# saidwivedi/TokenHMR

Measured on NVIDIA H100. Metric: images/sec (256x192) at bs=64 per GPU, full TokenHMR forward, higher is better.
Workload: dtype f16 operands / f32 accumulate

## Files before the change

tokenhmr_b200/_build.py:

```python
from __future__ import annotations

import hashlib
import os
import subprocess
import sys
from pathlib import Path

PKG_DIR = Path(__file__).resolve().parent
CSRC = PKG_DIR / "csrc"
LIB_PATH = PKG_DIR / "libtokenhmr_b200.so"
STAMP = PKG_DIR / ".libtokenhmr_b200.stamp"
PROBE_SRC = PKG_DIR.parent / "tests" / "csrc" / "kernel_probe.cu"
PROBE_PATH = PKG_DIR.parent / "tests" / "libthmr_probe.so"
PROBE_STAMP = PKG_DIR.parent / "tests" / ".libthmr_probe.stamp"
GEMM_PROBE_SRC = PKG_DIR.parent / "tests" / "csrc" / "gemm_probe.cu"
GEMM_PROBE_PATH = PKG_DIR.parent / "tests" / "libthmr_gemm_probe.so"
GEMM_PROBE_STAMP = PKG_DIR.parent / "tests" / ".libthmr_gemm_probe.stamp"

NVCC_FLAGS = [
    "-gencode", "arch=compute_90a,code=sm_90a",
    "-lineinfo", "-O3", "-std=c++17",
    "--expt-relaxed-constexpr",
    "-Xcompiler", "-fPIC", "-shared",
]
PROBE_FLAGS = ["-Xcompiler", "-fvisibility=hidden"]


def _nvcc() -> str:
    for cand in (os.environ.get("NVCC"), "/usr/local/cuda/bin/nvcc", "nvcc"):
        if cand and (os.path.isabs(cand) and os.path.exists(cand) or not os.path.isabs(cand)):
            return cand
    return "nvcc"


def source_hash(probe: bool = False) -> str:
    h = hashlib.sha256()
    files = sorted(CSRC.glob("*.cu")) + sorted(CSRC.glob("*.cuh")) + sorted((PKG_DIR.parent / "include").glob("*.h"))
    if probe:
        files += sorted(PROBE_SRC.parent.glob("*.cu"))
    for f in files:
# ... 3 lines not shown
    return h.hexdigest()


def _compile(src: Path, out: Path, stamp: Path, flags: list, want: str, force: bool, verbose: bool) -> Path:
    if not force and out.exists() and stamp.exists() and stamp.read_text().strip() == want:
        return out
    cmd = [_nvcc(), *flags, "-o", str(out), str(src)]
    if verbose:
        cmd.insert(1, "-Xptxas=-v")
        print(" ".join(cmd), file=sys.stderr)
    res = subprocess.run(cmd, capture_output=True, text=True)
    if res.returncode != 0:
        raise RuntimeError(f"nvcc failed ({res.returncode}):\n{res.stdout}\n{res.stderr}")
    if verbose:
        print(res.stderr, file=sys.stderr)
    stamp.write_text(want)
    return out


def build_probe(force: bool = False, verbose: bool = False) -> Path:
    if GEMM_PROBE_SRC.exists():
        _compile(GEMM_PROBE_SRC, GEMM_PROBE_PATH, GEMM_PROBE_STAMP, NVCC_FLAGS + PROBE_FLAGS, source_hash(probe=True),
                 force, verbose)
    return _compile(PROBE_SRC, PROBE_PATH, PROBE_STAMP, NVCC_FLAGS + PROBE_FLAGS, source_hash(probe=True), force,
                    verbose)


def build(force: bool = False, verbose: bool = False) -> Path:
    path = _compile(CSRC / "tokenhmr_b200.cu", LIB_PATH, STAMP, NVCC_FLAGS, source_hash(), force, verbose)
    if PROBE_SRC.exists():
        build_probe(force, verbose)
    return path


if __name__ == "__main__":
    print(build(force="--force" in sys.argv, verbose="-v" in sys.argv))
```

tokenhmr_b200/csrc/gemm_host.cuh:

```cuda
#pragma once
#include "common.cuh"

#include "gemm_wgmma.cuh"

namespace thmr {

struct GemmPlan {
  CUtensorMap tmA, tmB;
  CUtensorMap tmC;
  GemmParams p;
  int bn;
  int grid;
  int cluster;
  int fp8;
  int epi;
};

struct GemmDesc {
  const __half* A; int lda; long long a_rows;
  const __half* B; int ldb;
  int M, N, K;
  const float* bias = nullptr;
  const float* resid = nullptr; int ldr = 0; int resid_mod = 0;
  int act = kActNone; int act32 = 0;
  float* out32 = nullptr; int ld32 = 0;
  __half* out16 = nullptr; int ld16 = 0;
  int taps = 1; int cin = 0; int tap_row0 = 0; int tap_stride = 0;
  int seq_pitch = 0, seq_lo = 0, seq_hi = 0;
  float alpha = 1.0f;
  long long* argmin_out = nullptr; const float* row_sq = nullptr; const float* col_sq = nullptr;
  int* screen_rows = nullptr; int* screen_count = nullptr; const float* screen_cmax2 = nullptr;
  float screen_rel = 0.f, screen_abs = 0.f; int screen_row0 = 0;
  const int* row_map = nullptr; const int* m_dev = nullptr; int m_dev_off = 0;
  int force_bn = 0;
  int force_epi = 0;
  unsigned long long* stamp = nullptr;
  int fp8 = 0;
  const float* a_scale = nullptr; int ld_as = 0;
  const float* w_scale = nullptr;
  uint8_t* out8 = nullptr; int ld8 = 0; float* out8_scale = nullptr; int ld8s = 0;
};

inline int pick_bn(int M, int N, int K, bool staged_epilogue, int epi_kind, int force) {
  if (force) return force;
  const int sms = num_sms();
  const int tm = (M + kGemmBM - 1) / kGemmBM;
  const int num_kb = (K + kGemmBK - 1) / kGemmBK;
  int best = 256;
  double best_cost = -1;
  const int cands[4] = {256, 128, 64, 32};
  for (int i = 0; i < 4; ++i) {
    const int bn = cands[i];
    const long tiles = static_cast<long>(tm) * ((N + bn - 1) / bn);
    const long waves = (tiles + sms - 1) / sms;
    const double mma = 4.0 * bn;
    const double feed = (128.0 + bn) * 128.0 / 32.0;
    const double epilogue = !staged_epilogue                                 ? 0.0
                            : bn >= 128 && gemm_epi_tma_store(epi_kind)       ? 2500.0 * bn / 128
                            : bn >= 128 && epi_kind == kEpiBiasResidF32       ? 9000.0 * bn / 128
                            : bn == 256                                       ? 55000.0
                                                                              : 7000.0 * bn / 128;
    const double cost = waves * (num_kb * ((mma > feed ? mma : feed) + 40.0) + epilogue);
    if (best_cost < 0 || cost < best_cost) { best_cost = cost; best = bn; }
  }
  return best;
}

inline int pick_bn_fp8(int M, int N, int K) {
  const int sms = num_sms();
  const int tm = (M + kGemmBM - 1) / kGemmBM;
  const int num_kb = (K + 127) / 128;
  int best = 128;
  double best_cost = -1;
  const int cands[2] = {128, 64};
  for (int i = 0; i < 2; ++i) {
    const int bn = cands[i];
    const long tiles = static_cast<long>(tm) * ((N + bn - 1) / bn);
    const long waves = (tiles + sms - 1) / sms;
    const double mma = 4.0 * bn;
    const double feed = (128.0 + bn) * 128.0 / 32.0;
    const double cost = waves * (num_kb * ((mma > feed ? mma : feed) + bn + 40.0) + 7000.0 * bn / 128);
    if (best_cost < 0 || cost < best_cost) { best_cost = cost; best = bn; }
  }
  return best;
}

inline int gemm_pick_epi(const GemmDesc& d, int bn, int cluster) {
  auto al16 = [](const void* q) { return (reinterpret_cast<uintptr_t>(q) & 15) == 0; };
// ... 25 lines not shown
  THMR_CHECK(d.ld_as >= m_pad && d.ld_as % 4 == 0 && (reinterpret_cast<uintptr_t>(d.a_scale) & 15) == 0,
             "gemm fp8: activation scales need a 16-byte aligned [K/128][>= %ld] layout (ld_as %d)", m_pad, d.ld_as);
  int bn = d.force_bn ? d.force_bn : d.out8 ? 128 : pick_bn_fp8(d.M, d.N, d.K);
  THMR_CHECK(bn == 64 || bn == 128, "gemm fp8: block_n %d (64 or 128)", bn);
  THMR_CHECK(!d.out8 || (bn == 128 && d.out8_scale && d.ld8s >= d.M && !d.resid && !d.act32 && !d.seq_pitch),
             "gemm fp8: e4m3 output needs block_n 128, its scale array and no residual / mask / act32");
  GemmParams& p = plan->p;
  memset(&p, 0, sizeof(p));
  p.M = d.M; p.N = d.N; p.K = d.K;
  p.out32 = d.out32; p.ld32 = d.ld32; p.out16 = d.out16; p.ld16 = d.ld16;
  p.bias = d.bias; p.resid = d.resid; p.ldr = d.ldr; p.resid_mod = d.resid_mod; p.act = d.act; p.act32 = d.act32;
  p.seq_pitch = d.seq_pitch; p.seq_lo = d.seq_lo; p.seq_hi = d.seq_hi;
  p.alpha = d.alpha;
  p.stamp = d.stamp;
  p.kblocks_per_tap = d.K / 128;
  p.a_scale = d.a_scale; p.ld_as = d.ld_as; p.w_scale = d.w_scale;
  p.out8 = d.out8; p.ld8 = d.ld8; p.out8_scale = d.out8_scale; p.ld8s = d.ld8s;
  THMR_TRY(make_tmap_2d_e4m3(&plan->tmA, d.A, d.a_rows, d.K, d.lda, kGemmBM, 128));
  THMR_TRY(make_tmap_2d_e4m3(&plan->tmB, d.B, d.N, d.K, d.ldb, bn, 128));
  memset(&plan->tmC, 0, sizeof(plan->tmC));
  THMR_CHECK(d.force_epi == 0 || d.force_epi == 1 + kEpiGeneral, "gemm fp8: general epilogue only");
  plan->bn = bn;
  plan->cluster = 1;
  plan->fp8 = 1;
  plan->epi = kEpiGeneral;
  const long tiles_m = (d.M + kGemmBM - 1) / kGemmBM;
  const long tiles = tiles_m * ((d.N + bn - 1) / bn);
  p.m_fast = (tiles_m > 1 && d.M < d.N) ? 1 : 0;
  const long slots = num_sms();
  plan->grid = static_cast<int>(tiles < slots ? tiles : slots);
  return THMR_OK;
}

inline int gemm_make_plan(const GemmDesc& d, GemmPlan* plan) {
  if (d.fp8) return gemm_make_plan_fp8(d, plan);
  THMR_CHECK(d.M > 0 && d.N > 0 && d.K > 0, "gemm: bad shape %dx%dx%d", d.M, d.N, d.K);
  THMR_CHECK(d.out32 || d.out16 || d.argmin_out, "gemm: no output");
  const int cluster = d.force_bn == 512 ? 2 : 1;
  THMR_CHECK(cluster == 1 || !d.argmin_out, "gemm: block_n 512 (CTA pair) does not support the arg-min modes");
  const int kind = gemm_pick_epi(d, 256, cluster);
  const int bn = cluster == 2 ? 256 : pick_bn(d.M, d.N, d.K, d.argmin_out == nullptr, kind, d.force_bn);
  THMR_CHECK(bn == 32 || bn == 64 || bn == 128 || bn == 256, "gemm: bad block_n %d", bn);
  GemmParams& p = plan->p;
  memset(&p, 0, sizeof(p));
  p.M = d.M; p.N = d.N; p.K = d.K;
  p.out32 = d.out32; p.ld32 = d.ld32; p.out16 = d.out16; p.ld16 = d.ld16;
  p.bias = d.bias; p.resid = d.resid; p.ldr = d.ldr; p.resid_mod = d.resid_mod; p.act = d.act; p.act32 = d.act32;
  p.seq_pitch = d.seq_pitch; p.seq_lo = d.seq_lo; p.seq_hi = d.seq_hi;
  p.alpha = d.alpha; p.argmin_out = d.argmin_out; p.row_sq = d.row_sq; p.col_sq = d.col_sq;
  THMR_CHECK(!d.screen_rows || (d.argmin_out && d.screen_count && d.screen_cmax2),
             "gemm: screened arg-min needs its queue");
  THMR_CHECK((!d.m_dev && !d.row_map) || d.argmin_out, "gemm: device row count / row map are arg-min options");
  p.screen_rows = d.screen_rows; p.screen_count = d.screen_count; p.screen_cmax2 = d.screen_cmax2;
  p.screen_rel = d.screen_rel; p.screen_abs = d.screen_abs; p.screen_row0 = d.screen_row0;
  p.row_map = d.row_map; p.m_dev = d.m_dev; p.m_dev_off = d.m_dev_off;
  p.stamp = d.stamp;
  const int num_kb = (d.K + kGemmBK - 1) / kGemmBK;
  uint64_t a_cols = d.K;
  if (d.taps > 1) {
    THMR_CHECK(d.cin % kGemmBK == 0 && d.K == d.taps * d.cin, "gemm conv: cin %d taps %d K %d", d.cin, d.taps, d.K);
    p.kblocks_per_tap = d.cin / kGemmBK;
    p.tap_row0 = d.tap_row0; p.tap_stride = d.tap_stride;
    a_cols = d.cin;
  } else {
    p.kblocks_per_tap = num_kb;
  }
  THMR_TRY(make_tmap_2d_f16(&plan->tmA, d.A, d.a_rows, a_cols, d.lda, kGemmBM, kGemmBK, CU_TENSOR_MAP_SWIZZLE_128B));
  THMR_TRY(make_tmap_2d_f16(&plan->tmB, d.B, d.N, d.K, d.ldb, bn / cluster, kGemmBK, CU_TENSOR_MAP_SWIZZLE_128B));
  plan->bn = bn;
  plan->cluster = cluster;
  plan->fp8 = 0;
  plan->epi = gemm_pick_epi(d, bn, cluster);
  THMR_CHECK(d.force_epi == 0 || d.force_epi - 1 == kEpiGeneral || d.force_epi - 1 == plan->epi,
             "gemm: epilogue kind %d does not fit this GEMM (its kind is %d)", d.force_epi - 1, plan->epi);
  if (d.force_epi) plan->epi = d.force_epi - 1;
  memset(&plan->tmC, 0, sizeof(plan->tmC));
  if (gemm_epi_tma_store(plan->epi))
    THMR_TRY(make_tmap_2d_f16(&plan->tmC, d.out16, d.M, d.N, d.ld16, 64, 64, CU_TENSOR_MAP_SWIZZLE_128B));
  if (plan->epi == kEpiBiasResidF32)
    THMR_TRY(make_tmap_2d(&plan->tmC, CU_TENSOR_MAP_DATA_TYPE_FLOAT32, 4, d.out32, d.M, d.N, d.ld32, 64, 32,
                          CU_TENSOR_MAP_SWIZZLE_128B));
  const long tiles_m = (d.M + kGemmBM * cluster - 1) / (kGemmBM * cluster);
  const long tiles = d.argmin_out ? tiles_m : tiles_m * ((d.N + bn - 1) / bn);
  p.m_fast = (!d.argmin_out && tiles_m > 1 && d.M < d.N) ? 1 : 0;
  const long slots = num_sms() / cluster;
  plan->grid = cluster * static_cast<int>(tiles < slots ? tiles : slots);
  return THMR_OK;
}

template <int BN, int STAGES, int CLUSTER = 1, bool FP8 = false, int EPI = kEpiGeneral, bool TIMELINE = false>
inline int gemm_launch_t(const GemmPlan& plan, cudaStream_t stream) {
  using S = GemmSmem<BN, STAGES, FP8, EPI>;
  static_assert(S::kTotal <= kGemmSmemLimit, "GEMM shared memory exceeds 227 KB");
  static bool configured = false;
  if (!configured) {
    THMR_CUDA(cudaFuncSetAttribute(gemm_f16_tn_kernel<BN, STAGES, CLUSTER, FP8, EPI, TIMELINE>, cudaFuncAttributeMaxDynamicSharedMemorySize,
                                   S::kTotal));
    configured = true;
  }
  cudaLaunchConfig_t cfg = {};
  cfg.gridDim = dim3(plan.grid);
  cfg.blockDim = dim3(kGemmThreads);
  cfg.dynamicSmemBytes = S::kTotal;
  cfg.stream = stream;
  cudaLaunchAttribute attr[1];
  attr[0].id = cudaLaunchAttributeClusterDimension;
  attr[0].val.clusterDim.x = CLUSTER;
  attr[0].val.clusterDim.y = 1;
  attr[0].val.clusterDim.z = 1;
  cfg.attrs = attr;
  cfg.numAttrs = 1;
  THMR_CUDA(cudaLaunchKernelEx(&cfg, gemm_f16_tn_kernel<BN, STAGES, CLUSTER, FP8, EPI, TIMELINE>, plan.tmA, plan.tmB,
                               plan.tmC, plan.p));
  return THMR_OK;
}

template <int BN, int EPI>
constexpr int gemm_stages() {
  return BN == 256 ? 4 : EPI == kEpiBiasResidF32 ? 5 : 6;
}

template <int BN, bool TIMELINE>
inline int gemm_launch_epi(const GemmPlan& plan, cudaStream_t stream) {
  switch (plan.epi) {
    case kEpiGeneral: return gemm_launch_t<BN, gemm_stages<BN, kEpiGeneral>(), 1, false, kEpiGeneral, TIMELINE>(plan, stream);
    case kEpiF16: return gemm_launch_t<BN, gemm_stages<BN, kEpiF16>(), 1, false, kEpiF16, TIMELINE>(plan, stream);
    case kEpiBiasF16: return gemm_launch_t<BN, gemm_stages<BN, kEpiBiasF16>(), 1, false, kEpiBiasF16, TIMELINE>(plan, stream);
    case kEpiBiasGeluF16:
      return gemm_launch_t<BN, gemm_stages<BN, kEpiBiasGeluF16>(), 1, false, kEpiBiasGeluF16, TIMELINE>(plan, stream);
    case kEpiBiasResidF32:
      return gemm_launch_t<BN, gemm_stages<BN, kEpiBiasResidF32>(), 1, false, kEpiBiasResidF32, TIMELINE>(plan, stream);
  }
  return fail(THMR_ERR_INVALID, "gemm: unsupported epilogue kind %d", plan.epi);
}

inline int gemm_launch_plain(const GemmPlan& plan, cudaStream_t stream) {
  if (plan.fp8) {
    if (plan.bn == 128) return gemm_launch_t<128, 5, 1, true>(plan, stream);
    if (plan.bn == 64) return gemm_launch_t<64, 7, 1, true>(plan, stream);
    return fail(THMR_ERR_INVALID, "gemm fp8: unsupported block_n %d", plan.bn);
  }
  if (plan.cluster == 2) return gemm_launch_t<256, 4, 2>(plan, stream);
  switch (plan.bn) {
    case 256: return gemm_launch_epi<256, false>(plan, stream);
    case 128: return gemm_launch_epi<128, false>(plan, stream);
    case 64: return gemm_launch_t<64, 8>(plan, stream);
    case 32: return gemm_launch_t<32, 8>(plan, stream);
  }
  return fail(THMR_ERR_INVALID, "gemm: unsupported block_n %d", plan.bn);
}

template <bool TIMELINE = false>
inline int gemm_launch(const GemmPlan& plan, cudaStream_t stream) {
  if constexpr (TIMELINE) {
    THMR_CHECK(!plan.fp8 && plan.cluster == 1 && (plan.bn == 128 || plan.bn == 256),
               "gemm timeline: fp16 block_n 128 / 256 only (block_n %d)", plan.bn);
    return plan.bn == 256 ? gemm_launch_epi<256, true>(plan, stream) : gemm_launch_epi<128, true>(plan, stream);
  } else {
    THMR_CHECK(plan.epi == kEpiGeneral || (plan.bn >= 128 && plan.cluster == 1 && !plan.fp8),
               "gemm: epilogue kind %d at block_n %d", plan.epi, plan.bn);
    return gemm_launch_plain(plan, stream);
  }
}

}
```

tokenhmr_b200/csrc/gemm_wgmma.cuh:

```cuda
#pragma once
#include "common.cuh"
#include "ptx.cuh"

namespace thmr {

enum : int { kActNone = 0, kActGelu = 1, kActRelu = 2 };

enum : int { kEpiGeneral = 0, kEpiF16 = 1, kEpiBiasF16 = 2, kEpiBiasGeluF16 = 3, kEpiBiasResidF32 = 4 };

constexpr bool gemm_epi_tma_store(int epi) { return epi == kEpiF16 || epi == kEpiBiasF16 || epi == kEpiBiasGeluF16; }

struct GemmParams {
  int M, N, K;
  float* out32;
  int ld32;
  __half* out16;
  int ld16;
  const float* bias;
  const float* resid;
  int ldr;
  int resid_mod;
  int act;
  int act32;
  int kblocks_per_tap;
// ... 44 lines not shown
    if (m_stationary) {
      if (++n_blk == tiles_n) { n_blk = 0; m_blk += stride; }
    } else {
      tile += stride;
    }
  }
};

constexpr int kGemmBM = 128;
constexpr int kGemmBK = 64;
constexpr int kGemmConsumerWarps = 8;
constexpr int kGemmThreads = 32 * kGemmConsumerWarps + 128;
constexpr int kWarpTma = kGemmConsumerWarps;

template <int BN>
constexpr int gemm_chunk() { return BN == 64 || BN == 128 ? 64 : 32; }

template <bool FP8>
constexpr int gemm_bk() { return FP8 ? 128 : kGemmBK; }

constexpr uint32_t kGemmSmemLimit = 232448;
constexpr uint32_t kResidBoxBytes = 64 * 32 * 4;

template <int BN, int STAGES, bool FP8 = false, int EPI = kEpiGeneral>
struct GemmSmem {
  static constexpr uint32_t kABytes = kGemmBM * kGemmBK * 2;
  static constexpr uint32_t kBBytes = BN * kGemmBK * 2;
  static constexpr uint32_t kStageBytes = kABytes + kBBytes;
  static constexpr uint32_t kEpiOffset = STAGES * kStageBytes;
  static constexpr int kResidFit = static_cast<int>((kGemmSmemLimit - kEpiOffset - 256 - 1024) / (2 * kResidBoxBytes));
  static constexpr int kResidBufs = EPI != kEpiBiasResidF32 ? 0 : kResidFit < BN / 32 ? kResidFit : BN / 32;
  static_assert(EPI != kEpiBiasResidF32 || kResidBufs >= 2, "residual ring needs two boxes per warpgroup");
  static constexpr uint32_t kEpiWgBytes = EPI == kEpiBiasResidF32 ? kResidBufs * kResidBoxBytes : 64 * 128 * 2;
  static_assert(EPI == kEpiBiasResidF32 || 64 * gemm_chunk<BN>() * 4 <= kEpiWgBytes,
                "fp32 staging chunk exceeds the warpgroup's block");
  static constexpr uint32_t kEpiBytes = 2 * kEpiWgBytes;
  static constexpr uint32_t kScaleOffset = kEpiOffset + kEpiBytes;
  static constexpr uint32_t kScaleBytes = FP8 ? STAGES * kGemmBM * 4 : 0;
  static constexpr uint32_t kBarOffset = kScaleOffset + kScaleBytes;
  static_assert((2 * STAGES + 4 * kResidBufs) * 8 <= 256, "mbarriers exceed their 256 bytes");
  static constexpr uint32_t kRowScaleOffset = kBarOffset + 256;
  static constexpr uint32_t kRowScaleBytes = FP8 ? kGemmBM * 4 : 0;
  static constexpr uint32_t kTotal = kRowScaleOffset + kRowScaleBytes + 1024;
};

__device__ __forceinline__ float gelu_erf(float x) {
  const float a = fabsf(x) * 0.70710678118654752f;
  float p = fmaf(0.0000430638f, a, 0.0002765672f);
  p = fmaf(p, a, 0.0001520143f);
  p = fmaf(p, a, 0.0092705272f);
  p = fmaf(p, a, 0.0422820123f);
  p = fmaf(p, a, 0.0705230784f);
  p = fmaf(p, a, 1.0f);
  p *= p; p *= p; p *= p; p *= p;
  float r;
  asm("rcp.approx.ftz.f32 %0, %1;" : "=f"(r) : "f"(p));
// ... 169 lines not shown
#pragma unroll
          for (int e = 0; e < 4; ++e) h2[e] = __floats2half2_rn(v[2 * e], v[2 * e + 1]);
          *reinterpret_cast<uint4*>(o) = q;
        } else {
#pragma unroll
          for (int e = 0; e < 8; ++e)
            if (col + e < p.N) o[e] = __float2half_rn(v[e]);
        }
      }
    }
    named_barrier_sync(bar_id, 128);
  }
}

struct RingPos {
  int slot = 0;
  uint32_t phase = 0;
  template <int NB>
  __device__ __forceinline__ void next() {
    if (++slot == NB) { slot = 0; phase ^= 1; }
  }
};

template <int BN>
struct ResidBoxIter {
  TileIter it;
  int row_off, M, N, c = 0;
  __device__ ResidBoxIter(const TileIter& t, int ro, int m, int n) : it(t), row_off(ro), M(m), N(n) { skip(); }
  __device__ bool valid() const { return it.valid(); }
  __device__ int m0w() const { return it.m0(kGemmBM) + row_off; }
  __device__ int col() const { return it.n0(BN) + 32 * c; }
  __device__ void skip() {
    while (it.valid() && m0w() >= M) it.next();
  }
  __device__ void next() {
    if (++c == BN / 32 || col() >= N) {
      c = 0;
      it.next();
      skip();
    }
  }
};

template <int BN, int NB>
__device__ __forceinline__ void gemm_resid_thread(const CUtensorMap* tm, uint32_t ring, uint64_t* free_bar,
                                                  uint64_t* done, ResidBoxIter<BN> it) {
  for (int s = 0; s < NB; ++s) mbar_arrive(&free_bar[s]);
  RingPos rp;
  int prev = -1;
  for (; it.valid(); it.next()) {
    mbar_wait(&done[rp.slot], rp.phase);
    tma_reduce_add_2d(tm, ring + rp.slot * kResidBoxBytes, it.col(), it.m0w());
    tma_store_commit();
    if (prev >= 0) {
      tma_store_wait_read<1>();
      mbar_arrive(&free_bar[prev]);
    }
    prev = rp.slot;
    rp.next<NB>();
  }
  tma_store_wait<0>();
}

template <int BN, int NB>
__device__ __forceinline__ void gemm_epilogue_resid_tma(const GemmParams& p, const float (&acc)[BN / 2], uint32_t ring,
                                                        uint64_t* free_bar, uint64_t* done, RingPos& rp, int n0) {
  const int lane = threadIdx.x & 31;
  const int fr = ((threadIdx.x >> 5) & 3) * 16 + (lane >> 2);
  const int c0 = 2 * (lane & 3);
// ... 88 lines not shown
#pragma unroll
    for (int j = 0; j < BN / 8; ++j) {
#pragma unroll
      for (int c = 0; c < 2; ++c) {
        const int col = n0 + 8 * j + c0 + c;
        float v = acc[4 * j + 2 * i + c] * p.alpha;
        if (p.bias && col < p.N) v += __ldg(p.bias + col);
        v = gemm_act(p.act, v);
        acc[4 * j + 2 * i + c] = v;
        if (col < p.N) amax = fmaxf(amax, fabsf(v));
      }
    }
    amax = fmaxf(amax, __shfl_xor_sync(0xffffffffu, amax, 1));
    amax = fmaxf(amax, __shfl_xor_sync(0xffffffffu, amax, 2));
    const float s = e4m3_scale(amax);
    const int r = r0 + 8 * i;
    if ((threadIdx.x & 3) == 0) {
      sts_f32(row_inv + 4 * (r - wg * 64), 1.0f / s);
      if (m0 + r < M_eff) p.out8_scale[static_cast<size_t>(n0 / 128) * p.ld8s + m0 + r] = s;
    }
  }
}

template <int BN, int STAGES, int CLUSTER, bool FP8 = false, int EPI = kEpiGeneral, bool TIMELINE = false>
__global__ void __launch_bounds__(kGemmThreads, 1)
gemm_f16_tn_kernel(const __grid_constant__ CUtensorMap tmA, const __grid_constant__ CUtensorMap tmB,
                   const __grid_constant__ CUtensorMap tmC, const GemmParams p) {
  using S = GemmSmem<BN, STAGES, FP8, EPI>;
  constexpr int BK = gemm_bk<FP8>();
  constexpr int NB = S::kResidBufs;
  static_assert(BN == 32 || BN == 64 || BN == 128 || BN == 256, "BN must be a power of two in [32,256]");
  static_assert(CLUSTER == 1 || (CLUSTER == 2 && BN >= 128), "cluster pairs split B in two halves of >= 64 rows");
  static_assert(!FP8 || (CLUSTER == 1 && (BN == 64 || BN == 128)), "FP8: two accumulator sets fit at BN <= 128");
  static_assert(EPI == kEpiGeneral || (!FP8 && CLUSTER == 1 && BN >= 128), "epilogue kinds: fp16 BN 128 / 256 only");
  static_assert(!TIMELINE || (!FP8 && CLUSTER == 1), "timeline: fp16 single-CTA kernels only");

  extern __shared__ uint8_t smem_raw[];
  uint8_t* smem = reinterpret_cast<uint8_t*>((reinterpret_cast<uintptr_t>(smem_raw) + 1023) & ~uintptr_t(1023));
  uint64_t* full_bar = reinterpret_cast<uint64_t*>(smem + S::kBarOffset);
  uint64_t* empty_bar = full_bar + STAGES;
  uint64_t* rfree_bar = empty_bar + STAGES;
  uint64_t* rdone_bar = rfree_bar + 2 * NB;

  const int warp = threadIdx.x >> 5;
  const int lane = threadIdx.x & 31;

  int M_eff = p.M;
  if (p.m_dev != nullptr) {
    const int m = __ldg(p.m_dev) - p.m_dev_off;
    M_eff = m < 0 ? 0 : (m < p.M ? m : p.M);
  }
  constexpr int kRows = kGemmBM * CLUSTER;
  const int tiles_m = (M_eff + kRows - 1) / kRows;
  const int tiles_n = (p.N + BN - 1) / BN;
  const int num_kb = (p.K + BK - 1) / BK;
  const bool m_stationary = p.argmin_out != nullptr;
  const int rank = CLUSTER == 2 ? static_cast<int>(cluster_ctarank()) : 0;
  const int tile0 = static_cast<int>(blockIdx.x) / CLUSTER, tile_step = static_cast<int>(gridDim.x) / CLUSTER;

  stamp_start(p.stamp);
  if (threadIdx.x == 0) {
    for (int s = 0; s < STAGES; ++s) {
      mbar_init(&full_bar[s], 1);
      mbar_init(&empty_bar[s], kGemmConsumerWarps * CLUSTER);
    }
    for (int b = 0; b < 2 * NB; ++b) {
      mbar_init(&rfree_bar[b], 1);
      mbar_init(&rdone_bar[b], 4);
    }
    fence_mbar_init();
  }
  if (warp == kWarpTma && lane == 0) {
    tma_prefetch_desc(&tmA);
    tma_prefetch_desc(&tmB);
    if constexpr (gemm_epi_tma_store(EPI) || EPI == kEpiBiasResidF32) tma_prefetch_desc(&tmC);
  }
  if constexpr (CLUSTER == 2) cluster_sync_all();
  else __syncthreads();

  if (warp >= kWarpTma) {
    asm volatile("setmaxnreg.dec.sync.aligned.u32 40;");
    if (warp == kWarpTma && lane == 0) {
      int stage = 0;
      uint32_t phase = 0;
      for (TileIter it(tiles_m, tiles_n, m_stationary, p.m_fast != 0, tile0, tile_step); it.valid(); it.next()) {
        const int m0 = it.m0(kRows) + rank * kGemmBM;
        const int n0 = it.n0(BN);
        for (int kb = 0; kb < num_kb; ++kb) {
          if constexpr (CLUSTER == 2) mbar_wait_cluster(&empty_bar[stage], phase ^ 1);
          else mbar_wait(&empty_bar[stage], phase ^ 1);
          uint8_t* sa = smem + stage * S::kStageBytes;
          uint8_t* sb = sa + S::kABytes;
          const int tap = kb / p.kblocks_per_tap;
          const int kk = kb - tap * p.kblocks_per_tap;
          mbar_arrive_expect_tx(&full_bar[stage], S::kStageBytes + (FP8 ? kGemmBM * 4 : 0));
          tma_load_2d(sa, &tmA, &full_bar[stage], kk * BK, m0 + p.tap_row0 + tap * p.tap_stride);
          if constexpr (CLUSTER == 2)
            tma_load_2d_mcast(sb + rank * (BN / 2) * 128, &tmB, &full_bar[stage], kb * BK, n0 + rank * (BN / 2), 3);
          else
            tma_load_2d(sb, &tmB, &full_bar[stage], kb * BK, n0);
          if constexpr (FP8)
            bulk_load_1d(smem + S::kScaleOffset + stage * kGemmBM * 4, p.a_scale + static_cast<size_t>(kb) * p.ld_as + m0,
                         kGemmBM * 4, &full_bar[stage]);
          if (++stage == STAGES) { stage = 0; phase ^= 1; }
        }
      }
    }
    if constexpr (EPI == kEpiBiasResidF32) {
      const int rw = warp - kWarpTma - 1;
      if ((rw == 0 || rw == 1) && lane == 0)
        gemm_resid_thread<BN, NB>(
            &tmC, smem_u32(smem + S::kEpiOffset + rw * S::kEpiWgBytes), rfree_bar + rw * NB, rdone_bar + rw * NB,
            ResidBoxIter<BN>(TileIter(tiles_m, tiles_n, false, p.m_fast != 0, tile0, tile_step), 64 * rw, M_eff, p.N));
    }
    if constexpr (CLUSTER == 2) cluster_sync_all();
    return;
  }

  asm volatile("setmaxnreg.inc.sync.aligned.u32 232;");
  const int wg = warp >> 2;
  const uint32_t smem_base = smem_u32(smem);
  const bool vec_r = p.resid && p.ldr % 4 == 0 && aligned16(p.resid);
  const bool vec32 = p.out32 && p.ld32 % 4 == 0 && aligned16(p.out32);
  const bool vec16 = p.out16 && p.ld16 % 8 == 0 && aligned16(p.out16);
  const uint32_t epi_stage = smem_base + S::kEpiOffset + wg * S::kEpiWgBytes;
  const bool screen = p.argmin_out != nullptr && p.screen_rows != nullptr;
  const float m2a = -2.0f * p.alpha;
  const int r0 = wg * 64 + (warp & 3) * 16 + (lane >> 2);
  const int c0 = 2 * (lane & 3);
  float best[2] = {INFINITY, INFINITY}, second[2] = {INFINITY, INFINITY};
  int best_idx[2] = {0, 0};
  int stage = 0;
  uint32_t phase = 0;
  float acc[BN / 2];
  float tile[FP8 ? BN / 2 : 1];
  RingPos rp;

  auto release = [&](int s) {
    __syncwarp();
    if (lane == 0) {
      if constexpr (CLUSTER == 2) {
        mbar_arrive_cluster(&empty_bar[s], 0);
        mbar_arrive_cluster(&empty_bar[s], 1);
      } else {
        mbar_arrive(&empty_bar[s]);
      }
    }
  };
  auto stamp = [&](const TileIter& it, int k) {
    if (TIMELINE && p.timeline != nullptr && (threadIdx.x & 127) == 0) {
      const int slot = (it.tile - tile0) / tile_step;
      if (slot < p.timeline_slots)
        p.timeline[((static_cast<size_t>(blockIdx.x) * p.timeline_slots + slot) * 2 + wg) * 4 + k] = globaltimer();
    }
  };
  if (TIMELINE && p.timeline != nullptr && threadIdx.x == 0) p.timeline_sm[blockIdx.x] = static_cast<int>(smid());
  for (TileIter it(tiles_m, tiles_n, m_stationary, p.m_fast != 0, tile0, tile_step); it.valid(); it.next()) {
    const int m0 = it.m0(kRows) + rank * kGemmBM;
    const int n0 = it.n0(BN);
    int prev = -1;
    if constexpr (TIMELINE) stamp(it, 0);
    if constexpr (FP8) {
      const int r0l = r0 - wg * 64;
      const float* wsc = p.w_scale + static_cast<size_t>(n0 / 128) * num_kb;
#pragma unroll
      for (int a = 0; a < BN / 2; ++a) acc[a] = 0.f;
      for (int kb = 0; kb < num_kb; ++kb) {
        mbar_wait(&full_bar[stage], phase);
        const uint32_t sa = smem_base + stage * S::kStageBytes + wg * (64 * 128);
        const uint32_t sb = smem_base + stage * S::kStageBytes + S::kABytes;
        wgmma_fence_operand(tile);
// ... 115 lines not shown
```

tokenhmr_b200/csrc/ptx.cuh:

```cuda
#pragma once
#include <cuda.h>
#include <cuda_fp16.h>
#include <cuda_runtime.h>
#include <stdint.h>

namespace thmr {

__device__ unsigned int g_pipeline_timeout = 0;
constexpr uint32_t kSpinLimit = 1u << 24;

__device__ __forceinline__ uint32_t smem_u32(const void* p) {
  return static_cast<uint32_t>(__cvta_generic_to_shared(p));
}

__device__ __forceinline__ void sts_f32x2(uint32_t a, float x, float y) {
  asm volatile("st.shared.v2.f32 [%0], {%1, %2};" ::"r"(a), "f"(x), "f"(y));
}
__device__ __forceinline__ float4 lds_f32x4(uint32_t a) {
  float4 v;
  asm volatile("ld.shared.v4.f32 {%0, %1, %2, %3}, [%4];" : "=f"(v.x), "=f"(v.y), "=f"(v.z), "=f"(v.w) : "r"(a));
  return v;
}
__device__ __forceinline__ void sts_f32(uint32_t a, float x) { asm volatile("st.shared.f32 [%0], %1;" ::"r"(a), "f"(x)); }
__device__ __forceinline__ void sts_u32(uint32_t a, uint32_t x) { asm volatile("st.shared.b32 [%0], %1;" ::"r"(a), "r"(x)); }
__device__ __forceinline__ float lds_f32(uint32_t a) {
  float v;
  asm volatile("ld.shared.f32 %0, [%1];" : "=f"(v) : "r"(a));
  return v;
}
__device__ __forceinline__ void named_barrier_sync(uint32_t id, uint32_t threads) {
  asm volatile("bar.sync %0, %1;" ::"r"(id), "r"(threads) : "memory");
}

__device__ __forceinline__ unsigned long long globaltimer() {
  unsigned long long t;
  asm volatile("mov.u64 %0, %%globaltimer;" : "=l"(t));
  return t;
}
__device__ __forceinline__ uint32_t smid() {
  uint32_t s;
  asm volatile("mov.u32 %0, %%smid;" : "=r"(s));
  return s;
}

__device__ __forceinline__ uint32_t lane_id() {
  uint32_t l;
  asm volatile("mov.u32 %0, %%laneid;" : "=r"(l));
  return l;
}

__device__ __forceinline__ void mbar_init(uint64_t* bar, uint32_t count) {
  asm volatile("mbarrier.init.shared::cta.b64 [%0], %1;" ::"r"(smem_u32(bar)), "r"(count) : "memory");
}
__device__ __forceinline__ void fence_mbar_init() {
// ... 24 lines not shown
}
__device__ __forceinline__ bool mbar_wait(uint64_t* bar, uint32_t parity) {
#pragma unroll 1
  for (uint32_t it = 0; it < kSpinLimit; ++it) {
    if (mbar_try_wait(bar, parity)) return true;
  }
  atomicExch(&g_pipeline_timeout, 1u);
  return false;
}

__device__ __forceinline__ uint32_t cluster_ctarank() {
  uint32_t r;
  asm volatile("mov.u32 %0, %%cluster_ctarank;" : "=r"(r));
  return r;
}
__device__ __forceinline__ void cluster_sync_all() {
  asm volatile("barrier.cluster.arrive.release;\n\tbarrier.cluster.wait.acquire;" ::: "memory");
}
__device__ __forceinline__ void mbar_arrive_cluster(uint64_t* bar, uint32_t cta) {
  asm volatile(
      "{\n\t"
      ".reg .b32 ra;\n\t"
      "mapa.shared::cluster.u32 ra, %0, %1;\n\t"
      "mbarrier.arrive.release.cluster.shared::cluster.b64 _, [ra];\n\t"
      "}\n" ::"r"(smem_u32(bar)),
      "r"(cta)
      : "memory");
}
__device__ __forceinline__ bool mbar_wait_cluster(uint64_t* bar, uint32_t parity) {
#pragma unroll 1
  for (uint32_t it = 0; it < kSpinLimit; ++it) {
    uint32_t ok;
    asm volatile(
        "{\n\t"
        ".reg .pred P;\n\t"
        "mbarrier.try_wait.parity.acquire.cluster.shared::cta.b64 P, [%1], %2;\n\t"
        "selp.u32 %0, 1, 0, P;\n\t"
        "}\n"
        : "=r"(ok)
        : "r"(smem_u32(bar)), "r"(parity)
        : "memory");
    if (ok) return true;
  }
  atomicExch(&g_pipeline_timeout, 1u);
  return false;
}

// ... 130 lines not shown
```

Baseline: 1902.

## Add ping-pong warpgroup GEMM schedule on CTA pairs with cost-model selection

Adds a ping-pong consumer schedule in which the two consumer warpgroups each own alternating 128x128 tiles (two 64-row halves each). Named barriers pass the MMA turn between them, so one warpgroup's epilogue overlaps the other's main loop. The kernel runs as a 2-CTA cluster sharing B, and a cost model picks this schedule automatically for specialised epilogues when each CTA gets at least two tiles. It also drops the release qualifier from the cluster mbarrier arrive and retunes one epilogue cost constant. The risks are wrong schedule picks from the heuristic and weaker memory ordering on remote arrives.

Result: no change. 1887, median of 6 (-0.8%).

```diff
diff --git a/tokenhmr_b200/_build.py b/tokenhmr_b200/_build.py
--- a/tokenhmr_b200/_build.py
+++ b/tokenhmr_b200/_build.py
@@ -16,6 +16,9 @@
 GEMM_PROBE_SRC = PKG_DIR.parent / "tests" / "csrc" / "gemm_probe.cu"
 GEMM_PROBE_PATH = PKG_DIR.parent / "tests" / "libthmr_gemm_probe.so"
 GEMM_PROBE_STAMP = PKG_DIR.parent / "tests" / ".libthmr_gemm_probe.stamp"
+PP_PROBE_SRC = PKG_DIR.parent / "tests" / "csrc" / "gemm_pingpong_probe.cu"
+PP_PROBE_PATH = PKG_DIR.parent / "tests" / "libthmr_gemm_pingpong_probe.so"
+PP_PROBE_STAMP = PKG_DIR.parent / "tests" / ".libthmr_gemm_pingpong_probe.stamp"
 
 NVCC_FLAGS = [
     "-gencode", "arch=compute_90a,code=sm_90a",
@@ -65,6 +68,9 @@
     if GEMM_PROBE_SRC.exists():
         _compile(GEMM_PROBE_SRC, GEMM_PROBE_PATH, GEMM_PROBE_STAMP, NVCC_FLAGS + PROBE_FLAGS, source_hash(probe=True),
                  force, verbose)
+    if PP_PROBE_SRC.exists():
+        _compile(PP_PROBE_SRC, PP_PROBE_PATH, PP_PROBE_STAMP, NVCC_FLAGS + PROBE_FLAGS, source_hash(probe=True), force,
+                 verbose)
     return _compile(PROBE_SRC, PROBE_PATH, PROBE_STAMP, NVCC_FLAGS + PROBE_FLAGS, source_hash(probe=True), force,
                     verbose)
 
diff --git a/tokenhmr_b200/csrc/gemm_host.cuh b/tokenhmr_b200/csrc/gemm_host.cuh
--- a/tokenhmr_b200/csrc/gemm_host.cuh
+++ b/tokenhmr_b200/csrc/gemm_host.cuh
@@ -12,9 +12,12 @@
   int bn;
   int grid;
   int cluster;
+  int pingpong;
   int fp8;
   int epi;
 };
+
+enum : int { kSchedAuto = 0, kSchedCooperative = 1, kSchedPingPong = 2 };
 
 struct GemmDesc {
   const __half* A; int lda; long long a_rows;
@@ -34,6 +37,7 @@
   const int* row_map = nullptr; const int* m_dev = nullptr; int m_dev_off = 0;
   int force_bn = 0;
   int force_epi = 0;
+  int force_sched = 0;
   unsigned long long* stamp = nullptr;
   int fp8 = 0;
   const float* a_scale = nullptr; int ld_as = 0;
@@ -41,29 +45,46 @@
   uint8_t* out8 = nullptr; int ld8 = 0; float* out8_scale = nullptr; int ld8s = 0;
 };
 
-inline int pick_bn(int M, int N, int K, bool staged_epilogue, int epi_kind, int force) {
-  if (force) return force;
+inline double gemm_coop_cost(int M, int N, int K, bool staged_epilogue, int epi_kind, int bn) {
   const int sms = num_sms();
   const int tm = (M + kGemmBM - 1) / kGemmBM;
   const int num_kb = (K + kGemmBK - 1) / kGemmBK;
+  const long tiles = static_cast<long>(tm) * ((N + bn - 1) / bn);
+  const long waves = (tiles + sms - 1) / sms;
+  const double mma = 4.0 * bn;
+  const double feed = (128.0 + bn) * 128.0 / 32.0;
+  const double epilogue = !staged_epilogue                                 ? 0.0
+                          : bn >= 128 && gemm_epi_tma_store(epi_kind)       ? 2500.0 * bn / 128
+                          : bn >= 128 && epi_kind == kEpiBiasResidF32       ? 10000.0 * bn / 128
+                          : bn == 256                                       ? 55000.0
+                                                                            : 7000.0 * bn / 128;
+  return waves * (num_kb * ((mma > feed ? mma : feed) + 40.0) + epilogue);
+}
+
+inline int pick_bn(int M, int N, int K, bool staged_epilogue, int epi_kind, int force) {
+  if (force) return force;
   int best = 256;
   double best_cost = -1;
   const int cands[4] = {256, 128, 64, 32};
   for (int i = 0; i < 4; ++i) {
-    const int bn = cands[i];
-    const long tiles = static_cast<long>(tm) * ((N + bn - 1) / bn);
-    const long waves = (tiles + sms - 1) / sms;
-    const double mma = 4.0 * bn;
-    const double feed = (128.0 + bn) * 128.0 / 32.0;
-    const double epilogue = !staged_epilogue                                 ? 0.0
-                            : bn >= 128 && gemm_epi_tma_store(epi_kind)       ? 2500.0 * bn / 128
-                            : bn >= 128 && epi_kind == kEpiBiasResidF32       ? 9000.0 * bn / 128
-                            : bn == 256                                       ? 55000.0
-                                                                              : 7000.0 * bn / 128;
-    const double cost = waves * (num_kb * ((mma > feed ? mma : feed) + 40.0) + epilogue);
-    if (best_cost < 0 || cost < best_cost) { best_cost = cost; best = bn; }
+    const double cost = gemm_coop_cost(M, N, K, staged_epilogue, epi_kind, cands[i]);
+    if (best_cost < 0 || cost < best_cost) { best_cost = cost; best = cands[i]; }
   }
   return best;
+}
+
+inline bool pick_pingpong(int M, int N, int K, int epi_kind) {
+  if (epi_kind == kEpiGeneral) return false;
+  const long clusters = num_sms() / 2;
+  const long pairs = static_cast<long>((M + 2 * kGemmBM - 1) / (2 * kGemmBM)) * ((N + 127) / 128);
+  const long per_cta = (pairs + clusters - 1) / clusters;
+  if (per_cta < 2) return false;
+  const int num_kb = (K + kGemmBK - 1) / kGemmBK;
+  const double loop = num_kb * (1100.0 + 40.0);
+  const double epilogue = epi_kind == kEpiBiasResidF32 ? 17000.0 : 5000.0;
+  const double tile = loop > (loop + epilogue) / 2 ? loop : (loop + epilogue) / 2;
+  const double cost = per_cta * tile + epilogue;
+  return cost < gemm_coop_cost(M, N, K, true, epi_kind, pick_bn(M, N, K, true, epi_kind, 0));
 }
 
 inline int pick_bn_fp8(int M, int N, int K) {
@@ -135,6 +156,7 @@
   THMR_CHECK(d.force_epi == 0 || d.force_epi == 1 + kEpiGeneral, "gemm fp8: general epilogue only");
   plan->bn = bn;
   plan->cluster = 1;
+  plan->pingpong = 0;
   plan->fp8 = 1;
   plan->epi = kEpiGeneral;
   const long tiles_m = (d.M + kGemmBM - 1) / kGemmBM;
@@ -149,10 +171,16 @@
   if (d.fp8) return gemm_make_plan_fp8(d, plan);
   THMR_CHECK(d.M > 0 && d.N > 0 && d.K > 0, "gemm: bad shape %dx%dx%d", d.M, d.N, d.K);
   THMR_CHECK(d.out32 || d.out16 || d.argmin_out, "gemm: no output");
-  const int cluster = d.force_bn == 512 ? 2 : 1;
+  THMR_CHECK(d.force_sched >= kSchedAuto && d.force_sched <= kSchedPingPong, "gemm: bad schedule %d", d.force_sched);
+  const int kind = gemm_pick_epi(d, 256, 1);
+  const bool pp_fits = kind != kEpiGeneral && d.taps == 1 && (d.force_epi == 0 || d.force_epi - 1 == kind) &&
+                       (d.force_bn == 0 || d.force_bn == 128);
+  THMR_CHECK(d.force_sched != kSchedPingPong || pp_fits, "gemm: the ping-pong schedule does not fit this GEMM");
+  const bool pp = d.force_sched == kSchedPingPong ||
+                  (d.force_sched == kSchedAuto && d.force_bn == 0 && pp_fits && pick_pingpong(d.M, d.N, d.K, kind));
+  const int cluster = d.force_bn == 512 || pp ? 2 : 1;
   THMR_CHECK(cluster == 1 || !d.argmin_out, "gemm: block_n 512 (CTA pair) does not support the arg-min modes");
-  const int kind = gemm_pick_epi(d, 256, cluster);
-  const int bn = cluster == 2 ? 256 : pick_bn(d.M, d.N, d.K, d.argmin_out == nullptr, kind, d.force_bn);
+  const int bn = pp ? 128 : cluster == 2 ? 256 : pick_bn(d.M, d.N, d.K, d.argmin_out == nullptr, kind, d.force_bn);
   THMR_CHECK(bn == 32 || bn == 64 || bn == 128 || bn == 256, "gemm: bad block_n %d", bn);
   GemmParams& p = plan->p;
   memset(&p, 0, sizeof(p));
@@ -182,8 +210,9 @@
   THMR_TRY(make_tmap_2d_f16(&plan->tmB, d.B, d.N, d.K, d.ldb, bn / cluster, kGemmBK, CU_TENSOR_MAP_SWIZZLE_128B));
   plan->bn = bn;
   plan->cluster = cluster;
+  plan->pingpong = pp ? 1 : 0;
   plan->fp8 = 0;
-  plan->epi = gemm_pick_epi(d, bn, cluster);
+  plan->epi = pp ? kind : gemm_pick_epi(d, bn, cluster);
   THMR_CHECK(d.force_epi == 0 || d.force_epi - 1 == kEpiGeneral || d.force_epi - 1 == plan->epi,
              "gemm: epilogue kind %d does not fit this GEMM (its kind is %d)", d.force_epi - 1, plan->epi);
   if (d.force_epi) plan->epi = d.force_epi - 1;
@@ -201,14 +230,15 @@
   return THMR_OK;
 }
 
-template <int BN, int STAGES, int CLUSTER = 1, bool FP8 = false, int EPI = kEpiGeneral, bool TIMELINE = false>
+template <int BN, int STAGES, int CLUSTER = 1, bool FP8 = false, int EPI = kEpiGeneral, bool TIMELINE = false,
+          bool PP = false>
 inline int gemm_launch_t(const GemmPlan& plan, cudaStream_t stream) {
-  using S = GemmSmem<BN, STAGES, FP8, EPI>;
+  using S = GemmSmem<BN, STAGES, FP8, EPI, PP>;
   static_assert(S::kTotal <= kGemmSmemLimit, "GEMM shared memory exceeds 227 KB");
+  constexpr auto kernel = gemm_f16_tn_kernel<BN, STAGES, CLUSTER, FP8, EPI, TIMELINE, PP>;
   static bool configured = false;
   if (!configured) {
-    THMR_CUDA(cudaFuncSetAttribute(gemm_f16_tn_kernel<BN, STAGES, CLUSTER, FP8, EPI, TIMELINE>, cudaFuncAttributeMaxDynamicSharedMemorySize,
-                                   S::kTotal));
+    THMR_CUDA(cudaFuncSetAttribute(kernel, cudaFuncAttributeMaxDynamicSharedMemorySize, S::kTotal));
     configured = true;
   }
   cudaLaunchConfig_t cfg = {};
@@ -223,8 +253,7 @@
   attr[0].val.clusterDim.z = 1;
   cfg.attrs = attr;
   cfg.numAttrs = 1;
-  THMR_CUDA(cudaLaunchKernelEx(&cfg, gemm_f16_tn_kernel<BN, STAGES, CLUSTER, FP8, EPI, TIMELINE>, plan.tmA, plan.tmB,
-                               plan.tmC, plan.p));
+  THMR_CUDA(cudaLaunchKernelEx(&cfg, kernel, plan.tmA, plan.tmB, plan.tmC, plan.p));
   return THMR_OK;
 }
 
@@ -247,12 +276,24 @@
   return fail(THMR_ERR_INVALID, "gemm: unsupported epilogue kind %d", plan.epi);
 }
 
+template <bool TIMELINE>
+inline int gemm_launch_pingpong(const GemmPlan& plan, cudaStream_t stream) {
+  switch (plan.epi) {
+    case kEpiF16: return gemm_launch_t<128, 6, 2, false, kEpiF16, TIMELINE, true>(plan, stream);
+    case kEpiBiasF16: return gemm_launch_t<128, 6, 2, false, kEpiBiasF16, TIMELINE, true>(plan, stream);
+    case kEpiBiasGeluF16: return gemm_launch_t<128, 6, 2, false, kEpiBiasGeluF16, TIMELINE, true>(plan, stream);
+    case kEpiBiasResidF32: return gemm_launch_t<128, 6, 2, false, kEpiBiasResidF32, TIMELINE, true>(plan, stream);
+  }
+  return fail(THMR_ERR_INVALID, "gemm: no ping-pong kernel for epilogue kind %d", plan.epi);
+}
+
 inline int gemm_launch_plain(const GemmPlan& plan, cudaStream_t stream) {
   if (plan.fp8) {
     if (plan.bn == 128) return gemm_launch_t<128, 5, 1, true>(plan, stream);
     if (plan.bn == 64) return gemm_launch_t<64, 7, 1, true>(plan, stream);
     return fail(THMR_ERR_INVALID, "gemm fp8: unsupported block_n %d", plan.bn);
   }
+  if (plan.pingpong) return gemm_launch_pingpong<false>(plan, stream);
   if (plan.cluster == 2) return gemm_launch_t<256, 4, 2>(plan, stream);
   switch (plan.bn) {
     case 256: return gemm_launch_epi<256, false>(plan, stream);
@@ -266,11 +307,12 @@
 template <bool TIMELINE = false>
 inline int gemm_launch(const GemmPlan& plan, cudaStream_t stream) {
   if constexpr (TIMELINE) {
-    THMR_CHECK(!plan.fp8 && plan.cluster == 1 && (plan.bn == 128 || plan.bn == 256),
+    THMR_CHECK(!plan.fp8 && (plan.cluster == 1 || plan.pingpong) && (plan.bn == 128 || plan.bn == 256),
                "gemm timeline: fp16 block_n 128 / 256 only (block_n %d)", plan.bn);
+    if (plan.pingpong) return gemm_launch_pingpong<true>(plan, stream);
     return plan.bn == 256 ? gemm_launch_epi<256, true>(plan, stream) : gemm_launch_epi<128, true>(plan, stream);
   } else {
-    THMR_CHECK(plan.epi == kEpiGeneral || (plan.bn >= 128 && plan.cluster == 1 && !plan.fp8),
+    THMR_CHECK(plan.epi == kEpiGeneral || (plan.bn >= 128 && (plan.cluster == 1 || plan.pingpong) && !plan.fp8),
                "gemm: epilogue kind %d at block_n %d", plan.epi, plan.bn);
     return gemm_launch_plain(plan, stream);
   }
diff --git a/tokenhmr_b200/csrc/gemm_wgmma.cuh b/tokenhmr_b200/csrc/gemm_wgmma.cuh
--- a/tokenhmr_b200/csrc/gemm_wgmma.cuh
+++ b/tokenhmr_b200/csrc/gemm_wgmma.cuh
@@ -90,7 +90,7 @@
 constexpr uint32_t kGemmSmemLimit = 232448;
 constexpr uint32_t kResidBoxBytes = 64 * 32 * 4;
 
-template <int BN, int STAGES, bool FP8 = false, int EPI = kEpiGeneral>
+template <int BN, int STAGES, bool FP8 = false, int EPI = kEpiGeneral, bool PP = false>
 struct GemmSmem {
   static constexpr uint32_t kABytes = kGemmBM * kGemmBK * 2;
   static constexpr uint32_t kBBytes = BN * kGemmBK * 2;
@@ -100,6 +100,9 @@
   static constexpr int kResidBufs = EPI != kEpiBiasResidF32 ? 0 : kResidFit < BN / 32 ? kResidFit : BN / 32;
   static_assert(EPI != kEpiBiasResidF32 || kResidBufs >= 2, "residual ring needs two boxes per warpgroup");
   static constexpr uint32_t kEpiWgBytes = EPI == kEpiBiasResidF32 ? kResidBufs * kResidBoxBytes : 64 * 128 * 2;
+  static_assert(!PP || (BN == 128 && !FP8 && EPI != kEpiGeneral && STAGES * kStageBytes == 6 * 32768 &&
+                        kEpiWgBytes == 16384),
+                "ping-pong: 6 stages of 32 KB and 16 KB of staging or ring per warpgroup");
   static_assert(EPI == kEpiBiasResidF32 || 64 * gemm_chunk<BN>() * 4 <= kEpiWgBytes,
                 "fp32 staging chunk exceeds the warpgroup's block");
   static constexpr uint32_t kEpiBytes = 2 * kEpiWgBytes;
@@ -315,13 +318,15 @@
   }
 };
 
-template <int BN>
+template <int BN, int HALVES = 1>
 struct ResidBoxIter {
   TileIter it;
-  int row_off, M, N, c = 0;
-  __device__ ResidBoxIter(const TileIter& t, int ro, int m, int n) : it(t), row_off(ro), M(m), N(n) { skip(); }
+  int rows, row_off, M, N, c = 0, h = 0;
+  __device__ ResidBoxIter(const TileIter& t, int rw, int ro, int m, int n) : it(t), rows(rw), row_off(ro), M(m), N(n) {
+    skip();
+  }
   __device__ bool valid() const { return it.valid(); }
-  __device__ int m0w() const { return it.m0(kGemmBM) + row_off; }
+  __device__ int m0w() const { return it.m0(rows) + row_off + 64 * h; }
   __device__ int col() const { return it.n0(BN) + 32 * c; }
   __device__ void skip() {
     while (it.valid() && m0w() >= M) it.next();
@@ -329,15 +334,18 @@
   __device__ void next() {
     if (++c == BN / 32 || col() >= N) {
       c = 0;
-      it.next();
-      skip();
+      if (++h == HALVES || m0w() >= M) {
+        h = 0;
+        it.next();
+        skip();
+      }
     }
   }
 };
 
-template <int BN, int NB>
+template <int BN, int NB, int HALVES>
 __device__ __forceinline__ void gemm_resid_thread(const CUtensorMap* tm, uint32_t ring, uint64_t* free_bar,
-                                                  uint64_t* done, ResidBoxIter<BN> it) {
+                                                  uint64_t* done, ResidBoxIter<BN, HALVES> it) {
   for (int s = 0; s < NB; ++s) mbar_arrive(&free_bar[s]);
   RingPos rp;
   int prev = -1;
@@ -472,18 +480,96 @@
   }
 }
 
-template <int BN, int STAGES, int CLUSTER, bool FP8 = false, int EPI = kEpiGeneral, bool TIMELINE = false>
+constexpr uint32_t kBarMmaTurn = 3;
+
+template <int STAGES, int EPI, bool TIMELINE, typename Release>
+__device__ __forceinline__ void gemm_pingpong_consumer(const GemmParams& p, const CUtensorMap* tmC, uint32_t smem_base,
+                                                       uint64_t* full_bar, uint64_t* rfree_bar, uint64_t* rdone_bar,
+                                                       int tiles_m, int tiles_n, int num_kb, int M_eff, int rank,
+                                                       int tile0, int tile_step, Release release) {
+  constexpr int BN = 128;
+  using S = GemmSmem<BN, STAGES, false, EPI, true>;
+  constexpr int NB = S::kResidBufs;
+  const int wg = threadIdx.x >> 7;
+  const int num_tiles = (tiles_m * tiles_n - tile0 + tile_step - 1) / tile_step;
+  const uint32_t epi_stage = smem_base + S::kEpiOffset + wg * S::kEpiWgBytes;
+  float acc[2][BN / 2];
+  RingPos rp;
+  auto stamp = [&](int t, int k) {
+    if (TIMELINE && p.timeline != nullptr && (threadIdx.x & 127) == 0 && t < p.timeline_slots)
+      p.timeline[((static_cast<size_t>(blockIdx.x) * p.timeline_slots + t) * 2 + wg) * 4 + k] = globaltimer();
+  };
+  if (TIMELINE && p.timeline != nullptr && threadIdx.x == 0) p.timeline_sm[blockIdx.x] = static_cast<int>(smid());
+  int t = wg;
+  for (TileIter it(tiles_m, tiles_n, false, p.m_fast != 0, tile0 + wg * tile_step, 2 * tile_step); it.valid();
+       it.next(), t += 2) {
+    const int m0 = it.m0(2 * kGemmBM) + rank * kGemmBM;
+    const int n0 = it.n0(BN);
+    if constexpr (TIMELINE) stamp(t, 0);
+    if (t > 0) named_barrier_sync(kBarMmaTurn + wg, 256);
+    const int e = t * num_kb;
+    int stage = e % STAGES;
+    uint32_t phase = (e / STAGES) & 1;
+    int prev = -1;
+    for (int kb = 0; kb < num_kb; ++kb) {
+      mbar_wait(&full_bar[stage], phase);
+      if constexpr (TIMELINE) if (kb == 0) stamp(t, 1);
+      const uint32_t sa = smem_base + stage * S::kStageBytes;
+      const uint32_t sb = sa + S::kABytes;
+      wgmma_fence_operand(acc[0]);
+      wgmma_fence_operand(acc[1]);
+      wgmma_fence();
+#pragma unroll
+      for (int k = 0; k < kGemmBK / 16; ++k) {
+#pragma unroll
+        for (int h = 0; h < 2; ++h)
+          wgmma_tile_k16<BN>(acc[h], make_wgmma_desc_sw128(sa + h * (64 * 128) + k * 32),
+                             make_wgmma_desc_sw128(sb + k * 32), (kb | k) != 0 ? 1u : 0u);
+      }
+      wgmma_commit();
+      wgmma_wait<1>();
+      wgmma_fence_operand(acc[0]);
+      wgmma_fence_operand(acc[1]);
+      if (prev >= 0) release(prev);
+      prev = stage;
+      if (++stage == STAGES) { stage = 0; phase ^= 1; }
+    }
+    if (t + 1 < num_tiles) named_barrier_arrive(kBarMmaTurn + (wg ^ 1), 256);
+    wgmma_wait<0>();
+    wgmma_fence_operand(acc[0]);
+    wgmma_fence_operand(acc[1]);
+    if constexpr (TIMELINE) stamp(t, 2);
+    release(prev);
+#pragma unroll
+    for (int h = 0; h < 2; ++h) {
+      if constexpr (EPI == kEpiBiasResidF32) {
+        if (m0 + 64 * h < M_eff)
+          gemm_epilogue_resid_tma<BN, NB>(p, acc[h], epi_stage, rfree_bar + wg * NB, rdone_bar + wg * NB, rp, n0);
+      } else {
+        gemm_epilogue_f16_tma<BN, EPI>(p, acc[h], tmC, epi_stage, m0 + 64 * h, n0, M_eff, 1 + wg);
+      }
+    }
+    if constexpr (TIMELINE) stamp(t, 3);
+  }
+  if constexpr (gemm_epi_tma_store(EPI))
+    if ((threadIdx.x & 127) == 0) tma_store_wait<0>();
+}
+
+template <int BN, int STAGES, int CLUSTER, bool FP8 = false, int EPI = kEpiGeneral, bool TIMELINE = false,
+          bool PP = false>
 __global__ void __launch_bounds__(kGemmThreads, 1)
 gemm_f16_tn_kernel(const __grid_constant__ CUtensorMap tmA, const __grid_constant__ CUtensorMap tmB,
                    const __grid_constant__ CUtensorMap tmC, const GemmParams p) {
-  using S = GemmSmem<BN, STAGES, FP8, EPI>;
+  using S = GemmSmem<BN, STAGES, FP8, EPI, PP>;
   constexpr int BK = gemm_bk<FP8>();
   constexpr int NB = S::kResidBufs;
   static_assert(BN == 32 || BN == 64 || BN == 128 || BN == 256, "BN must be a power of two in [32,256]");
   static_assert(CLUSTER == 1 || (CLUSTER == 2 && BN >= 128), "cluster pairs split B in two halves of >= 64 rows");
   static_assert(!FP8 || (CLUSTER == 1 && (BN == 64 || BN == 128)), "FP8: two accumulator sets fit at BN <= 128");
-  static_assert(EPI == kEpiGeneral || (!FP8 && CLUSTER == 1 && BN >= 128), "epilogue kinds: fp16 BN 128 / 256 only");
-  static_assert(!TIMELINE || (!FP8 && CLUSTER == 1), "timeline: fp16 single-CTA kernels only");
+  static_assert(EPI == kEpiGeneral || (!FP8 && (CLUSTER == 1 || PP) && BN >= 128),
+                "epilogue kinds: fp16 BN 128 / 256 only");
+  static_assert(!PP || (CLUSTER == 2 && BN == 128 && EPI != kEpiGeneral), "ping-pong: specialised kinds, CTA pairs");
+  static_assert(!TIMELINE || (!FP8 && (CLUSTER == 1 || PP)), "timeline: fp16 single-CTA or ping-pong kernels only");
 
   extern __shared__ uint8_t smem_raw[];
   uint8_t* smem = reinterpret_cast<uint8_t*>((reinterpret_cast<uintptr_t>(smem_raw) + 1023) & ~uintptr_t(1023));
@@ -512,7 +598,7 @@
   if (threadIdx.x == 0) {
     for (int s = 0; s < STAGES; ++s) {
       mbar_init(&full_bar[s], 1);
-      mbar_init(&empty_bar[s], kGemmConsumerWarps * CLUSTER);
+      mbar_init(&empty_bar[s], (PP ? 4 : kGemmConsumerWarps) * CLUSTER);
     }
     for (int b = 0; b < 2 * NB; ++b) {
       mbar_init(&rfree_bar[b], 1);
@@ -558,10 +644,20 @@
     }
     if constexpr (EPI == kEpiBiasResidF32) {
       const int rw = warp - kWarpTma - 1;
-      if ((rw == 0 || rw == 1) && lane == 0)
-        gemm_resid_thread<BN, NB>(
-            &tmC, smem_u32(smem + S::kEpiOffset + rw * S::kEpiWgBytes), rfree_bar + rw * NB, rdone_bar + rw * NB,
-            ResidBoxIter<BN>(TileIter(tiles_m, tiles_n, false, p.m_fast != 0, tile0, tile_step), 64 * rw, M_eff, p.N));
+      if ((rw == 0 || rw == 1) && lane == 0) {
+        const uint32_t ring = smem_u32(smem + S::kEpiOffset + rw * S::kEpiWgBytes);
+        if constexpr (PP)
+          gemm_resid_thread<BN, NB, 2>(
+              &tmC, ring, rfree_bar + rw * NB, rdone_bar + rw * NB,
+              ResidBoxIter<BN, 2>(TileIter(tiles_m, tiles_n, false, p.m_fast != 0, tile0 + rw * tile_step,
+                                           2 * tile_step),
+                                  kRows, rank * kGemmBM, M_eff, p.N));
+        else
+          gemm_resid_thread<BN, NB, 1>(
+              &tmC, ring, rfree_bar + rw * NB, rdone_bar + rw * NB,
+              ResidBoxIter<BN>(TileIter(tiles_m, tiles_n, false, p.m_fast != 0, tile0, tile_step), kGemmBM, 64 * rw,
+                               M_eff, p.N));
+      }
     }
     if constexpr (CLUSTER == 2) cluster_sync_all();
     return;
@@ -597,6 +693,12 @@
       }
     }
   };
+  if constexpr (PP) {
+    gemm_pingpong_consumer<STAGES, EPI, TIMELINE>(p, &tmC, smem_base, full_bar, rfree_bar, rdone_bar, tiles_m, tiles_n,
+                                                  num_kb, M_eff, rank, tile0, tile_step, release);
+    cluster_sync_all();
+    return;
+  }
   auto stamp = [&](const TileIter& it, int k) {
     if (TIMELINE && p.timeline != nullptr && (threadIdx.x & 127) == 0) {
       const int slot = (it.tile - tile0) / tile_step;
diff --git a/tokenhmr_b200/csrc/ptx.cuh b/tokenhmr_b200/csrc/ptx.cuh
--- a/tokenhmr_b200/csrc/ptx.cuh
+++ b/tokenhmr_b200/csrc/ptx.cuh
@@ -30,6 +30,9 @@
 }
 __device__ __forceinline__ void named_barrier_sync(uint32_t id, uint32_t threads) {
   asm volatile("bar.sync %0, %1;" ::"r"(id), "r"(threads) : "memory");
+}
+__device__ __forceinline__ void named_barrier_arrive(uint32_t id, uint32_t threads) {
+  asm volatile("bar.arrive %0, %1;" ::"r"(id), "r"(threads) : "memory");
 }
 
 __device__ __forceinline__ unsigned long long globaltimer() {
@@ -100,7 +103,7 @@
       "{\n\t"
       ".reg .b32 ra;\n\t"
       "mapa.shared::cluster.u32 ra, %0, %1;\n\t"
-      "mbarrier.arrive.release.cluster.shared::cluster.b64 _, [ra];\n\t"
+      "mbarrier.arrive.shared::cluster.b64 _, [ra];\n\t"
       "}\n" ::"r"(smem_u32(bar)),
       "r"(cta)
       : "memory");
```
